# solvithrastar/MultiMesh

Hardware: AMD Instinct MI355X
Metric: interpolated points/sec, 10M->10M 3D mesh, 1 scalar field (higher is better)
Workload: dtype f64; 1 GPU; metric: hex8 3D 10077696 source nodes -> 10077696 targets in all, 10077696 on rank 0 (n_src=216, n_tgt=216 per side, jittered unit cube), 1 field component(s), k=20; targets: ONE 216^3 = 10077696-node target mesh (jitter seed 7); targets_per_gpu=10077696, targets_total=10077696, knn_kernel=lane, parallelism=single GPU

## Files before the change

### include/multimesh_hip.h

```cpp
#ifndef MULTIMESH_HIP_H
#define MULTIMESH_HIP_H

#include <stddef.h>
#include <stdint.h>

#ifdef __cplusplus
extern "C" {
#endif

#define MM_OK 0
#define MM_ERR_ARG (-1)
#define MM_ERR_HIP (-2)
#define MM_ERR_NODEVICE (-3)
#define MM_ERR_ALLOC (-4)
#define MM_ERR_UNSUPPORTED (-5)

#define MM_KNN_MAX_K 64


void centroid(long long ndim, long long nelem, long long npointsperelem,
              long long *connectivity, double *points, double *centroid);

long long triLinearInterpolator(long long nelem_to_search, long long npoints,
                                long long *nearest_element_indices, long long *connectivity,
// ... 129 lines not shown

int64_t mm_interpolate_hex8(mm_context *ctx, const double *nodes_d, int64_t nnodes,
                            const int64_t *connectivity_d, int64_t nelem, const double *points_d,
                            int64_t npoints, const double *fields_d, int64_t ncomp,
                            int64_t nelem_to_search, double *out_d, int64_t *enc_d, double *w_d);

typedef struct mm_source mm_source;
int mm_source_create(mm_context *ctx, const double *nodes_d, int64_t nnodes, const int64_t *connectivity_d, int64_t nelem,
                     mm_source **out);
void mm_source_destroy(mm_context *ctx, mm_source *source);
int64_t mm_interpolate_hex8_on(mm_context *ctx, const mm_source *source, const double *points_d, int64_t npoints,
                               const double *fields_d, int64_t ncomp, int64_t nelem_to_search, double *out_d,
                               int64_t *enc_d, double *w_d);

int64_t mm_interpolate_hex8_host(mm_context *ctx, const double *nodes_h, int64_t nnodes,
                                 const int64_t *connectivity_h, int64_t nelem, const double *points_h,
                                 int64_t npoints, const double *fields_h, int64_t ncomp,
                                 int64_t nelem_to_search, double *out_h, int64_t *enc_h, double *w_h);

int mm_set_lazy_lists(mm_context *ctx, int on);

#define MM_FP_EXACT 0
#define MM_FP_TOL 1
int mm_set_fp_mode(mm_context *ctx, int mode);
int mm_get_fp_mode(mm_context *ctx);
int mm_last_locate_stats(mm_context *ctx, long long *out4);
#define MM_KNN_RAN_LANE 1
#define MM_KNN_RAN_STRIP 2
#define MM_KNN_RAN_CELL 4
#define MM_KNN_RAN_LIST 8
#define MM_KNN_RAN_GENERIC 16
#define MM_KNN_RAN_LEVELS 32
#define MM_KNN_RAN_TREE 64
int mm_last_knn_kernels(mm_context *ctx, int *mask);

enum mm_stage {
    MM_STAGE_CENTROID = 0,
    MM_STAGE_KNN_BUILD = 1,
    MM_STAGE_KNN_QUERY = 2,
    MM_STAGE_LOCATE = 3,
    MM_STAGE_GATHER = 4,
    MM_STAGE_KNN_CELL = 5,
    MM_STAGE_LOCATE_PASS0 = 6,
    MM_STAGE_COUNT = 7
};
int mm_set_profiling(mm_context *ctx, int on);
int mm_last_timings(mm_context *ctx, double *ms, int n);

#ifdef __cplusplus
}
#endif
#endif
```

### multimesh_amd/csrc/mm_centroid.hip

```cpp
#include "mm_common.h"

template <int NDIM, int NPER>
__global__ __launch_bounds__(256) void centroid_kernel(i64 nelem, i64 nper_rt,
                                                       const i64 *__restrict__ conn,
                                                       const double *__restrict__ points,
                                                       double *__restrict__ out)
{
    const i64 e = (i64)blockIdx.x * blockDim.x + threadIdx.x;
    if (e >= nelem) return;
    const i64 nper = NPER > 0 ? NPER : nper_rt;
    const i64 *row = conn + e * nper;
    double acc[NDIM];
#pragma unroll
    for (int a = 0; a < NDIM; ++a) acc[a] = 0.;
    if (NPER > 0) {
        i64 id[NPER > 0 ? NPER : 1];
#pragma unroll
        for (int p = 0; p < NPER; ++p) id[p] = row[p];
#pragma unroll
        for (int p = 0; p < NPER; ++p) {
#pragma unroll
            for (int a = 0; a < NDIM; ++a) acc[a] = acc[a] + points[id[p] * NDIM + a];
        }
    } else {
        for (i64 p = 0; p < nper; ++p) {
            const i64 id = row[p];
#pragma unroll
            for (int a = 0; a < NDIM; ++a) acc[a] = acc[a] + points[id * NDIM + a];
        }
    }
    const double denom = (double)nper;
#pragma unroll
    for (int a = 0; a < NDIM; ++a) out[e * NDIM + a] = acc[a] / denom;
// ... 25 lines not shown
        double acc[3] = {0., 0., 0.};
#pragma unroll
        for (int p = 0; p < 8; ++p) {
#pragma unroll
            for (int a = 0; a < 3; ++a) acc[a] = acc[a] + points[id[p] * 3 + a];
        }
#pragma unroll
        for (int a = 0; a < 3; ++a) {
            const double c = acc[a] / 8.0;
            out[e * 3 + a] = c;
            mn[a] = fmin(mn[a], c);
            mx[a] = fmax(mx[a], c);
        }
    }
#pragma unroll
    for (int a = 0; a < 3; ++a)
        for (int off = 32; off > 0; off >>= 1) {
            mn[a] = fmin(mn[a], __shfl_xor(mn[a], off));
            mx[a] = fmax(mx[a], __shfl_xor(mx[a], off));
        }
    const int wave = threadIdx.x >> 6;
    if ((threadIdx.x & 63) == 0)
#pragma unroll
        for (int a = 0; a < 3; ++a) {
            s_box[a][wave] = mn[a];
            s_box[3 + a][wave] = mx[a];
        }
    __syncthreads();
    if (threadIdx.x < 6) {
        double v = s_box[threadIdx.x][0];
        for (int w = 1; w < 256 / 64; ++w) v = threadIdx.x < 3 ? fmin(v, s_box[threadIdx.x][w]) : fmax(v, s_box[threadIdx.x][w]);
        partial[(i64)blockIdx.x * 6 + threadIdx.x] = v;
    }
}

int mm_launch_centroid_bbox(mm_context *ctx, i64 nelem, const i64 *conn, const double *points, double *out,
                            double *partial, int nblocks)
{
    if (nelem == 0) return MM_OK;
    hipLaunchKernelGGL(centroid_bbox_kernel, dim3((unsigned)nblocks), dim3(256), 0, ctx->stream, nelem, conn, points,
                       out, partial);
    MM_HIP_CHECK(hipGetLastError());
    return MM_OK;
}

int mm_launch_centroid(mm_context *ctx, i64 ndim, i64 nelem, i64 nper, const i64 *conn,
                       const double *points, double *out)
{
    if (nelem == 0) return MM_OK;
    const int block = 256;
    const i64 grid = (nelem + block - 1) / block;
    MM_REQUIRE(grid < (i64)0x7fffffff, "too many elements for one launch");
    dim3 g((unsigned)grid), b(block);
    if (ndim == 3 && nper == 8)
        hipLaunchKernelGGL((centroid_kernel<3, 8>), g, b, 0, ctx->stream, nelem, nper, conn, points, out);
    else if (ndim == 3)
        hipLaunchKernelGGL((centroid_kernel<3, 0>), g, b, 0, ctx->stream, nelem, nper, conn, points, out);
    else if (ndim == 2 && nper == 4)
        hipLaunchKernelGGL((centroid_kernel<2, 4>), g, b, 0, ctx->stream, nelem, nper, conn, points, out);
    else if (ndim == 2)
        hipLaunchKernelGGL((centroid_kernel<2, 0>), g, b, 0, ctx->stream, nelem, nper, conn, points, out);
    else
        hipLaunchKernelGGL((centroid_kernel<1, 0>), g, b, 0, ctx->stream, nelem, nper, conn, points, out);
    MM_HIP_CHECK(hipGetLastError());
    return MM_OK;
}
// ... 16 lines not shown
```

### multimesh_amd/csrc/mm_common.h

```cpp
#pragma once

#include <hip/hip_runtime.h>
#include <stdint.h>
#include <stdio.h>

#include "multimesh_hip.h"

typedef long long i64;

void mm_set_error(int code, const char *fmt, ...);

#define MM_HIP_CHECK(expr)                                                              \
    do {                                                                                \
        hipError_t _e = (expr);                                                         \
        if (_e != hipSuccess) {                                                         \
            mm_set_error(MM_ERR_HIP, "%s:%d: %s -> %s", __FILE__, __LINE__, #expr,      \
                         hipGetErrorString(_e));                                        \
            return MM_ERR_HIP;                                                          \
        }                                                                               \
    } while (0)

#define MM_REQUIRE(cond, msg)                                                           \
    do {                                                                                \
        if (!(cond)) {                                                                  \
// ... 37 lines not shown
    MM_BUF_L_PTS,
    MM_BUF_LOC_SLOW,
    MM_BUF_TREE_KEYS,
    MM_BUF_TREE_XYZ,
    MM_BUF_TREE_LEVEL,
    MM_BUF_TREE_COARSE,
    MM_BUF_TREE_DOWN,
    MM_BUF_LEVELS,
    MM_BUF_SAMPLE_POINTS = MM_BUF_LEVELS + 2 * 8,
    MM_BUF_COUNT
};

struct mm_context {
    int device = 0;
    hipStream_t stream = nullptr;
    mm_scratch scratch;
    void *buf_ptr[MM_BUF_COUNT] = {};
    size_t buf_cap[MM_BUF_COUNT] = {};
    i64 *d_counters = nullptr;
    i64 *h_counters = nullptr;
    int profiling = 0;
    int lazy_lists = 1;
    int fp_mode = 0;
    hipEvent_t ev_begin[MM_STAGE_COUNT];
    hipEvent_t ev_end[MM_STAGE_COUNT];
    bool ev_used[MM_STAGE_COUNT];
    bool ev_created = false;
    hipEvent_t ev_misc = nullptr;
    struct {
        bool valid = false;
        i64 nsrc = 0;
        double box[6] = {0, 0, 0, 0, 0, 0};
        int stat_shift = -1;
        int misses = 0;
        long long calls_guessed = 0;
    } grid_guess;
    struct {
        bool valid = false;
        i64 npts = 0, ncells = 0;
        bool dense = false;
    } lane_hint;
    int knn_kernels = 0;
    int *abort_flags = nullptr;
    hipStream_t copy_stream = nullptr;
    hipEvent_t ev_copy[3] = {nullptr, nullptr, nullptr};
};

int mm_scratch_begin(mm_context *ctx, size_t total);
void *mm_scratch_take(mm_context *ctx, size_t bytes);
static inline size_t mm_round256(size_t b) { return (b + 255) & ~(size_t)255; }
static inline size_t mm_fill_span(size_t b) { return mm_guard_alloc() ? b : mm_round256(b); }

int mm_zero_async(mm_context *ctx, void *dst_d, size_t bytes);

int mm_mirror_async(mm_context *ctx, long long *dst_pinned, const long long *src_d, int n);

int mm_buffer_get(mm_context *ctx, int slot, size_t bytes, void **out);

void mm_stage_reset(mm_context *ctx);
void mm_stage_begin(mm_context *ctx, int stage);
void mm_stage_end(mm_context *ctx, int stage);

constexpr int kMmStatSlot = 32, kMmBoxSlot = 48, kMmAbortSlot = 24;

__device__ __forceinline__ bool mm_aborted(const int *__restrict__ abort6)
{
    if (!abort6) return false;
    const int4 a = *reinterpret_cast<const int4 *>(abort6);
    const int2 b = *reinterpret_cast<const int2 *>(abort6 + 4);
    return (a.x | a.y | a.z | a.w | b.x | b.y) != 0;
}

int mm_launch_centroid(mm_context *ctx, i64 ndim, i64 nelem, i64 nper, const i64 *conn,
                       const double *points, double *out);
int mm_launch_centroid_bbox(mm_context *ctx, i64 nelem, const i64 *conn, const double *points, double *out,
                            double *partial, int nblocks);
struct mm_knn_index;
struct mm_lazy_lists {
    const mm_knn_index *index;
    i64 k_full;
    int *nn_full;
};
int mm_launch_locate_hex8(mm_context *ctx, i64 k, i64 npoints, const void *nn, bool nn_is_int32,
                          const i64 *conn, i64 nelem, int conn_is_exodus, i64 *enc, const double *nodes,
                          double *w, const double *pts, i64 *d_nfailed, int zero_failed,
                          const double *fields, i64 nnodes, i64 ncomp, double *out,
                          const mm_lazy_lists *lazy, const double *tsorted = nullptr);
#define MM_LONG_LIST_MIN 32768
int mm_knn_query_list_impl(mm_context *ctx, const mm_knn_index *ix, const double *pts_d, i64 npts, i64 k,
                           int *idx_d, const int *list, const int *list_count, i64 list_len_hint);
int mm_launch_gather(mm_context *ctx, const double *fields, i64 nsrc, i64 ncomp, const i64 *ids,
                     const double *w, i64 npoints, i64 P, double *out, int out_point_major);

struct mm_knn_tree {
    double lo[3] = {0, 0, 0};
    double size = 1.0;
    double scale = 1.0;
    unsigned long long *keys = nullptr;
    double *xyz = nullptr;
    unsigned char *level = nullptr;
    int *coarse = nullptr;
    bool borrowed = false;
};
// ... 17 lines not shown
```

### multimesh_amd/csrc/mm_knn.hip

```cpp
#include <math.h>
#include <stdlib.h>

#include <new>
#include <type_traits>

#include "mm_common.h"
#include <cstring>

int mm_exclusive_scan_int(mm_context *ctx, const int *counts, i64 n, int *start, int *tile_sums);
size_t mm_radix_sort_scratch(i64 n);
int mm_radix_sort_pairs(mm_context *ctx, unsigned long long *ka, unsigned long long *kb, unsigned *va, unsigned *vb, i64 n,
                        int first_shift, int end_shift, void *scratch, bool *in_a);

namespace {
#include "mm_knn_grid.inc.h"
#include "mm_knn_rings.inc.h"
#include "mm_knn_tiles.inc.h"
#include "mm_knn_tree.inc.h"
#include "mm_knn_lane.inc.h"

__global__ __launch_bounds__(kBlock) void target_scatter_kernel(const int *__restrict__ rank_of, i64 npts,
                                                                const double *__restrict__ pts, int ndim, GridParams g,
                                                                const int *__restrict__ start,
                                                                double *__restrict__ tsorted,
                                                                const int *__restrict__ list,
                                                                const int *__restrict__ list_count)
{
    const i64 t = (i64)blockIdx.x * blockDim.x + threadIdx.x;
    if (t >= (list ? (i64)*list_count : npts)) return;
    const i64 p = list ? (i64)list[t] : t;
    const double x = pts[p * ndim], y = ndim > 1 ? pts[p * ndim + 1] : 0.0, z = ndim > 2 ? pts[p * ndim + 2] : 0.0;
    const i64 pos = (i64)start[cell_of_point(x, y, z, g)] + rank_of[t];
    store_record(tsorted + pos * kRec, x, y, z, (int)p);
}

constexpr int kLaneMaxK = 20;
struct LaneWork {
    int Z;
    int T, W;
// ... 298 lines not shown
{
    const unsigned gpts = (unsigned)((npts + kBlock - 1) / kBlock);
    const int ntiles = (int)((ncells + kScanTile - 1) / kScanTile);
    if (!list && ncells <= kHistCells && npts >= 64 * ncells)
        hipLaunchKernelGGL(cell_count_hist_kernel, dim3(256), dim3(kHistBlock), 0, ctx->stream, pts_d, npts, ndim, gl,
                           (int)ncells, cell_of, counts);
    else
        hipLaunchKernelGGL(cell_count_kernel, dim3(gpts), dim3(kBlock), 0, ctx->stream, pts_d, npts, ndim, gl, cell_of,
                           counts, list, list_count);
    hipLaunchKernelGGL(scan_tile_sums_kernel, dim3(ntiles), dim3(kBlock), 0, ctx->stream, counts, ncells, tile_sums,
                       (unsigned long long *)nullptr, 0);
    launch_scan_tail(ctx, counts, ncells, tile_sums, ntiles, start);
    hipLaunchKernelGGL(target_scatter_kernel, dim3(gpts), dim3(kBlock), 0, ctx->stream, cell_of, npts, pts_d, ndim, gl,
                       start, tsorted, list, list_count);
    MM_HIP_CHECK(hipGetLastError());
    return MM_OK;
}

static int build_level(mm_context *ctx, const double *src_d, i64 nsrc, int ndim, const double *box, double per_cell,
                       bool use_context_buffers, int level, int *level_extra, mm_knn_index **out,
                       double *sparse_share = nullptr, bool stat_dirty = true, const GuessedBuild *guessed = nullptr)
{
    static_assert(kMaxLevels - 1 <= 8, "mm_buffer_slot reserves 8 pairs for the denser levels");
    const int slot_cells = level == 0 ? (int)MM_BUF_CELL_START : (int)MM_BUF_LEVELS + 2 * (level - 1);
    const int slot_xyz = level == 0 ? (int)MM_BUF_SORTED_XYZ : (int)MM_BUF_LEVELS + 2 * (level - 1) + 1;
    *out = nullptr;
    mm_knn_index *ix = new (std::nothrow) mm_knn_index();
    if (!ix) {
        mm_set_error(MM_ERR_ALLOC, "out of host memory");
        return MM_ERR_ALLOC;
    }
    ix->nsrc = nsrc;
    ix->ndim = ndim;
    int live = 0;
    grid_layout(box, nsrc, ndim, per_cell, ix, &live);
    const i64 ncells = ix->ncells;
    const GridParams g = params_of(ix);

    hipError_t e = hipSuccess;
    if (use_context_buffers) {
        ix->borrowed = true;
        int brc = mm_buffer_get(ctx, slot_cells, (size_t)(ncells + 1) * sizeof(int), (void **)&ix->cell_start);
        if (brc == MM_OK)
            brc = mm_buffer_get(ctx, slot_xyz, (size_t)(nsrc + 1) * kRec * sizeof(double), (void **)&ix->sorted_xyz);
        if (brc != MM_OK) {
            free_index(ix);
            return brc;
        }
    } else {
        e = mm_raw_alloc(ctx->device, (void **)&ix->cell_start, (size_t)(ncells + 1) * sizeof(int));
        if (e == hipSuccess)
            e = mm_raw_alloc(ctx->device, (void **)&ix->sorted_xyz, (size_t)(nsrc + 1) * kRec * sizeof(double));
        if (e != hipSuccess) {
            mm_set_error(MM_ERR_ALLOC, "kNN index allocation failed: %s", hipGetErrorString(e));
            free_index(ix);
            return MM_ERR_ALLOC;
        }
    }
    const int ntiles = (int)((ncells + kScanTile - 1) / kScanTile);
    size_t need = mm_round256((size_t)(nsrc > 0 ? nsrc : 1) * sizeof(int)) +
                  mm_round256((size_t)(ncells + 1) * sizeof(int)) +
                  mm_round256((size_t)ntiles * sizeof(int)) + 4096;
    int rc = mm_scratch_begin(ctx, need);
    if (rc != MM_OK) { free_index(ix); return rc; }
    int *cell_of = (int *)mm_scratch_take(ctx, (size_t)(nsrc > 0 ? nsrc : 1) * sizeof(int));
    int *counts = (int *)mm_scratch_take(ctx, (size_t)(ncells + 1) * sizeof(int));
    int *tile_sums = (int *)mm_scratch_take(ctx, (size_t)ntiles * sizeof(int));
    if (!cell_of || !counts || !tile_sums) {
        mm_set_error(MM_ERR_ALLOC, "scratch carve failed");
        free_index(ix);
        return MM_ERR_ALLOC;
    }
    rc = mm_zero_async(ctx, counts, mm_fill_span((size_t)(ncells + 1) * sizeof(int)));
    if (rc != MM_OK) { free_index(ix); return rc; }
    const unsigned gsrc = (unsigned)((nsrc + kBlock - 1) / kBlock);
    if (guessed)
        {
            GuessBox gb6;
            for (int q = 0; q < 6; ++q) gb6.v[q] = box[q];
            hipLaunchKernelGGL(bbox_final_kernel, dim3(6), dim3(kBlock), 0, ctx->stream, guessed->box_partial, guessed->box_nblocks,
                               reinterpret_cast<double *>(ctx->h_counters + kBoxSlot),
                               reinterpret_cast<long long *>(ctx->d_counters + kStatSlot), gb6,
                               reinterpret_cast<int *>(ctx->d_counters + kMmAbortSlot));
        }
    if (nsrc > 0)
        hipLaunchKernelGGL(cell_count_kernel, dim3(gsrc), dim3(kBlock), 0, ctx->stream, src_d, nsrc, ndim, g, cell_of,
                           counts, (const int *)nullptr, (const int *)nullptr);
    const bool want_stat = level_extra != nullptr && nsrc >= kLevelMinSources && live > 0;
    const int sample_shift = (ncells + kBlock - 1) / kBlock >= 1024 ? 4 : 0;
    if (level_extra) *level_extra = 0;
    i64 *stat = ctx->d_counters + kStatSlot;
    if (want_stat && stat_dirty) e = hipMemsetAsync(stat, 0, 16 * sizeof(i64), ctx->stream);
    if (e == hipSuccess)
        hipLaunchKernelGGL(scan_tile_sums_kernel, dim3(ntiles), dim3(kBlock), 0, ctx->stream, counts, ncells, tile_sums,
                           want_stat ? (unsigned long long *)stat : (unsigned long long *)nullptr, sample_shift);
    launch_scan_tail(ctx, counts, ncells, tile_sums, ntiles, ix->cell_start,
                     want_stat ? (const long long *)stat : (const long long *)nullptr,
                     (long long *)(ctx->h_counters + kStatSlot), want_stat ? kMaxLevels : 0);
    if (want_stat) {
        if (e == hipSuccess) e = hipEventRecord(ctx->ev_misc, ctx->stream);
        if (e != hipSuccess) {
            mm_set_error(MM_ERR_HIP, "grid statistic: %s", hipGetErrorString(e));
            free_index(ix);
            return MM_ERR_HIP;
        }
    }
    if (nsrc > 0)
        hipLaunchKernelGGL(cell_scatter_kernel, dim3(gsrc), dim3(kBlock), 0, ctx->stream, src_d, nsrc, ndim, g, cell_of,
                           ix->cell_start, ix->sorted_xyz);
    e = hipGetLastError();
    if (e != hipSuccess) {
        mm_set_error(MM_ERR_HIP, "kNN build launch: %s", hipGetErrorString(e));
        free_index(ix);
        return MM_ERR_HIP;
    }
    if (guessed) *guessed->stat_shift = want_stat ? sample_shift : -1;
// ... 74 lines not shown
    {
        const int mode = tree_mode();
        bool cube = ndim == 3 && nsrc >= kLevelMinSources;
        for (int a = 0; a < 3 && cube; ++a) cube = box[3 + a] - box[a] > 0.0 && isfinite(box[3 + a] - box[a]);
        const bool deepest = (extra & (1 << (kMaxLevels - 2))) != 0, mesh_graded = (box_partial_d != nullptr || hex8_centroids) && extra != 0;
        if (cube && (mode == 1 || (mode == -1 && (deepest || mesh_graded) && max_levels > 1))) {
            rc = tree_build(ctx, head, src_d, nsrc, box, use_context_buffers);
            if (rc != MM_OK) {
                free_index(head);
                return rc;
            }
            extra = 0x10000;
        }
    }
    mm_knn_index *tail = head;
    for (int l = 1; l < max_levels; ++l) {
        per_cell /= kLevelRatio;
        if (!(extra & (1 << (l - 1)))) continue;
        if ((double)nsrc / per_cell > (double)kLevelMaxCells) break;
        mm_knn_index *lvl = nullptr;
        rc = build_level(ctx, src_d, nsrc, (int)ndim, box, per_cell, use_context_buffers, l, nullptr, &lvl);
        if (rc != MM_OK) {
            free_index(head);
            return rc;
        }
        tail->fine = lvl;
        tail = lvl;
    }
    *out = head;
    if (use_context_buffers && box_partial_d && ndim == 3) {
        ctx->grid_guess.valid = !head->fine && extra == 0 && per_cell_level0 == kDefaultPerCell && max_levels > 1;
        ctx->grid_guess.nsrc = nsrc;
        for (int q = 0; q < 6; ++q) ctx->grid_guess.box[q] = box[q];
    }
    return MM_OK;
}

int mm_knn_build_guessed(mm_context *ctx, const double *cen, i64 nelem, const double *box_partial, int box_nblocks,
                         mm_knn_index **out)
{
    *out = nullptr;
    GuessedBuild gb;
    gb.box_partial = box_partial;
    gb.box_nblocks = box_nblocks;
    gb.stat_shift = &ctx->grid_guess.stat_shift;
    int extra = 0;
    double sparse = 0.0;
    return build_level(ctx, cen, nelem, 3, ctx->grid_guess.box, kDefaultPerCell, true, 0, &extra, out, &sparse,
                       false, &gb);
}

bool mm_knn_guess_confirmed(mm_context *ctx)
{
    const double *h_box = reinterpret_cast<const double *>(ctx->h_counters + kBoxSlot);
    if (memcmp(h_box, ctx->grid_guess.box, 6 * sizeof(double)) != 0) return false;
    if (ctx->grid_guess.stat_shift < 0) return true;
    double sparse_count = 0.0;
    const int extra = stat_verdict(ctx, ctx->grid_guess.nsrc, ctx->grid_guess.stat_shift, &sparse_count);
    return extra == 0 && !(sparse_count / (double)ctx->grid_guess.nsrc > kSparseShare);
}


static TreeParams tree_params_of(const mm_knn_tree *tr)
{
    TreeParams tp;
    tp.lox = tr->lo[0];
    tp.loy = tr->lo[1];
    tp.loz = tr->lo[2];
    tp.scale = tr->scale;
    tp.size = tr->size;
    return tp;
}

static int tree_mode()
{
    const char *env = getenv("MM_KNN_TREE");
    return env ? (atoi(env) == 0 ? 0 : 1) : -1;
}

static int tree_build(mm_context *ctx, mm_knn_index *ix, const double *src_d, i64 nsrc, const double *box,
                      bool use_context_buffers)
{
    mm_knn_tree *tr = new (std::nothrow) mm_knn_tree();
    if (!tr) {
        mm_set_error(MM_ERR_ALLOC, "out of host memory");
        return MM_ERR_ALLOC;
    }
    double ext = 0.0;
// ... 486 lines not shown
```

### multimesh_amd/csrc/mm_knn_grid.inc.h

```cpp


constexpr int kBlock = 256;
constexpr double kDefaultPerCell = 8.0;
constexpr int kMaxCellsPerAxis = 1024;
constexpr double kLevelRatio = 2.0;
constexpr int kMaxLevels = 9;
constexpr int kLevelCount[kMaxLevels - 1] = {15, 19, 38, 77, 154, 307, 614, 1229};
constexpr double kLevelShare = 0.02;
constexpr int kSparseCount = 5;
constexpr double kSparseShare = 0.25;
constexpr i64 kLevelMinSources = 4096;
constexpr i64 kLevelMaxCells = (i64)1 << 27;
constexpr int kListKeepMax = 24;
constexpr i64 kLongListMin = MM_LONG_LIST_MIN;
constexpr int kSplitTargets = 128;
constexpr int kMaxSplit = 64;
constexpr int kStatSlot = kMmStatSlot;
static_assert(kMaxLevels <= 16, "the level statistic has 16 counter slots");
constexpr int kBoxSlot = kMmBoxSlot;

struct GridParams {
    int nx, ny, nz;
    double lox, loy, loz;
    double hx, hy, hz;
    double ihx, ihy, ihz;
};

__global__ __launch_bounds__(kBlock) void bbox_partial_kernel(const double *__restrict__ src, i64 nsrc,
                                                              int ndim, double *__restrict__ partial)
{
    __shared__ double smin[3][kBlock / 64];
    __shared__ double smax[3][kBlock / 64];
    double mn[3] = {INFINITY, INFINITY, INFINITY};
    double mx[3] = {-INFINITY, -INFINITY, -INFINITY};
    for (i64 e = (i64)blockIdx.x * blockDim.x + threadIdx.x; e < nsrc; e += (i64)gridDim.x * blockDim.x) {
        for (int a = 0; a < ndim; ++a) {
            const double v = src[e * ndim + a];
            mn[a] = fmin(mn[a], v);
            mx[a] = fmax(mx[a], v);
        }
    }
    for (int a = 0; a < 3; ++a) {
        for (int off = 32; off > 0; off >>= 1) {
            mn[a] = fmin(mn[a], __shfl_xor(mn[a], off));
            mx[a] = fmax(mx[a], __shfl_xor(mx[a], off));
        }
    }
    const int wave = threadIdx.x >> 6;
    if ((threadIdx.x & 63) == 0)
        for (int a = 0; a < 3; ++a) {
            smin[a][wave] = mn[a];
            smax[a][wave] = mx[a];
        }
    __syncthreads();
    if (threadIdx.x == 0) {
        for (int a = 0; a < 3; ++a) {
            double lo = smin[a][0], hi = smax[a][0];
            for (int wv = 1; wv < kBlock / 64; ++wv) {
                lo = fmin(lo, smin[a][wv]);
                hi = fmax(hi, smax[a][wv]);
            }
            partial[blockIdx.x * 6 + a] = lo;
            partial[blockIdx.x * 6 + 3 + a] = hi;
        }
    }
}

struct GuessBox {
    double v[6];
};
__global__ __launch_bounds__(kBlock) void bbox_final_kernel(const double *__restrict__ partial, int nblocks,
                                                             double *__restrict__ out, long long *__restrict__ stat16,
                                                             GuessBox guess = GuessBox(), int *__restrict__ mismatch6 = nullptr)
{
    __shared__ double s_part[kBlock / 64];
    const int a = blockIdx.x;
    if (stat16 && a == 0 && threadIdx.x < 16) stat16[threadIdx.x] = 0;
    const double init = a < 3 ? INFINITY : -INFINITY;
    double v[8];
#pragma unroll
    for (int u = 0; u < 8; ++u) v[u] = init;
    for (int b = threadIdx.x; b < nblocks; b += 8 * kBlock) {
#pragma unroll
        for (int u = 0; u < 8; ++u) {
            const int bb = b + kBlock * u;
            const double p = bb < nblocks ? partial[bb * 6 + a] : init;
            v[u] = a < 3 ? fmin(v[u], p) : fmax(v[u], p);
        }
    }
    double r = init;
#pragma unroll
    for (int u = 0; u < 8; ++u) r = a < 3 ? fmin(r, v[u]) : fmax(r, v[u]);
    for (int off = 32; off > 0; off >>= 1) {
        const double o = __shfl_xor(r, off);
        r = a < 3 ? fmin(r, o) : fmax(r, o);
    }
    if ((threadIdx.x & 63) == 0) s_part[threadIdx.x >> 6] = r;
    __syncthreads();
    if (threadIdx.x == 0) {
        for (int wv = 1; wv < kBlock / 64; ++wv) r = a < 3 ? fmin(r, s_part[wv]) : fmax(r, s_part[wv]);
        out[a] = r;
        if (mismatch6) mismatch6[a] = r == guess.v[a] ? 0 : 1;
    }
}

__device__ __forceinline__ int cell_coord(double x, double lo, double ih, int n)
{
    double t = (x - lo) * ih;
    t = fmin(fmax(t, 0.0), (double)(n - 1));
    return (int)t;
}

__device__ __forceinline__ int count_and_rank(int c, bool live, int *__restrict__ counts)
{
    const int lane = threadIdx.x & 63;
    const int prev = __shfl_up(c, 1);
    const bool head = lane == 0 || c != prev;
    const unsigned long long heads = __ballot(head);
    const unsigned long long upto = heads & (~0ull >> (63 - lane));
    const int head_lane = 63 - __clzll((long long)upto);
    const unsigned long long after = lane == 63 ? 0ull : heads & (~0ull << (lane + 1));
    int base = 0;
    if (head && live) {
        const int next_head = after ? __ffsll((long long)after) - 1 : 64;
        base = atomicAdd(&counts[c], next_head - lane);
    }
    base = __shfl(base, head_lane);
    return base + (lane - head_lane);
}

__device__ __forceinline__ int cell_of_point(double x, double y, double z, const GridParams &g)
{
    const int cx = cell_coord(x, g.lox, g.ihx, g.nx);
    const int cy = cell_coord(y, g.loy, g.ihy, g.ny);
    const int cz = cell_coord(z, g.loz, g.ihz, g.nz);
    return (cx * g.ny + cy) * g.nz + cz;
}

__global__ __launch_bounds__(kBlock) void cell_count_kernel(const double *__restrict__ src, i64 nsrc, int ndim,
                                                            GridParams g, int *__restrict__ rank_of,
                                                            int *__restrict__ counts, const int *__restrict__ list,
                                                            const int *__restrict__ list_count)
{
    const i64 e = (i64)blockIdx.x * blockDim.x + threadIdx.x;
    const bool live = e < (list ? (i64)*list_count : nsrc);
    int c = -1;
    if (live) {
        const i64 p = list ? (i64)list[e] : e;
        c = cell_of_point(src[p * ndim], ndim > 1 ? src[p * ndim + 1] : 0.0, ndim > 2 ? src[p * ndim + 2] : 0.0, g);
    }
    const int rank = count_and_rank(c, live, counts);
    if (live) rank_of[e] = rank;
}

constexpr int kHistBlock = 1024;
constexpr int kHistCells = 16384;
__global__ __launch_bounds__(kHistBlock) void cell_count_hist_kernel(const double *__restrict__ src, i64 nsrc, int ndim,
                                                                     GridParams g, int ncells, int *__restrict__ rank_of,
                                                                     int *__restrict__ counts)
{
    __shared__ int s_bin[kHistCells];
    for (int t = threadIdx.x; t < ncells; t += kHistBlock) s_bin[t] = 0;
    __syncthreads();
    const i64 chunks = (nsrc + kHistBlock - 1) / kHistBlock;
    const i64 c_lo = chunks * blockIdx.x / gridDim.x, c_hi = chunks * (blockIdx.x + 1) / gridDim.x;
    for (i64 ch = c_lo; ch < c_hi; ++ch) {
        const i64 e = ch * kHistBlock + threadIdx.x;
        const bool live = e < nsrc;
        int c = -1;
// ... 128 lines not shown
        s += v[i];
    }
    int total;
    int excl = block_exclusive_scan(s, &total) + tile_base;
    for (int i = 0; i < kScanItems; ++i) {
        if (base + i < n) start[base + i] = excl;
        excl += v[i];
    }
    if (blockIdx.x == gridDim.x - 1 && threadIdx.x == kBlock - 1) start[n] = excl;
}

__global__ __launch_bounds__(kBlock) void scan_apply_kernel(const int *__restrict__ counts, i64 n,
                                                            const int *__restrict__ tile_offsets,
                                                            int *__restrict__ start)
{
    const i64 base = (i64)blockIdx.x * kScanTile + (i64)threadIdx.x * kScanItems;
    int v[kScanItems];
    int s = 0;
    for (int i = 0; i < kScanItems; ++i) {
        v[i] = base + i < n ? counts[base + i] : 0;
        s += v[i];
    }
    int total;
    int excl = block_exclusive_scan(s, &total) + tile_offsets[blockIdx.x];
    for (int i = 0; i < kScanItems; ++i) {
        if (base + i < n) {
            start[base + i] = excl;
        }
        excl += v[i];
    }
    if (blockIdx.x == gridDim.x - 1 && threadIdx.x == kBlock - 1) start[n] = excl;
}

constexpr int kRec = 4;

__device__ __forceinline__ void store_record(double *__restrict__ rec, double x, double y, double z, int id)
{
    double2 *r2 = reinterpret_cast<double2 *>(rec);
    r2[0] = make_double2(x, y);
    r2[1] = make_double2(z, __longlong_as_double((long long)id));
}

__device__ __forceinline__ int record_id(double w) { return (int)__double_as_longlong(w); }

__global__ __launch_bounds__(kBlock) void cell_scatter_kernel(const double *__restrict__ src, i64 nsrc, int ndim,
                                                              GridParams g, const int *__restrict__ rank_of,
                                                              const int *__restrict__ start,
                                                              double *__restrict__ sorted_rec)
{
    const i64 e = (i64)blockIdx.x * blockDim.x + threadIdx.x;
    if (e >= nsrc) return;
    const double x = src[e * ndim], y = ndim > 1 ? src[e * ndim + 1] : 0.0, z = ndim > 2 ? src[e * ndim + 2] : 0.0;
    const i64 pos = (i64)start[cell_of_point(x, y, z, g)] + rank_of[e];
    store_record(sorted_rec + pos * kRec, x, y, z, (int)e);
}


constexpr int kWave = 64;
constexpr int kHistBuckets = 64;
constexpr int kTileCap = 256;
constexpr int kMaxGroups = 8;
constexpr int kSlots = kTileCap / kMaxGroups;

__device__ __forceinline__ int group_scan(int v, int sl, int S)
{
    for (int d = 1; d < S; d <<= 1) {
        const int t = __shfl_up(v, d, S);
        if (sl >= d) v += t;
    }
    return v;
}

__device__ __forceinline__ void wave_sync()
{
    __builtin_amdgcn_fence(__ATOMIC_RELEASE, "wavefront");
    __builtin_amdgcn_wave_barrier();
    __builtin_amdgcn_fence(__ATOMIC_ACQUIRE, "wavefront");
// ... 2 lines not shown
```

### multimesh_amd/csrc/mm_pipeline.hip

```cpp
#include <cstdlib>
#include <mutex>
#include <new>

#include "mm_common.h"

int mm_knn_build_impl(mm_context *ctx, const double *src_d, i64 nsrc, i64 ndim, mm_knn_index **out,
                      bool use_context_buffers, const double *box_partial_d, int box_nblocks, bool hex8_centroids = false);
int mm_knn_query_impl(mm_context *ctx, const mm_knn_index *ix, const double *pts_d, i64 npts, i64 k, void *idx_d,
                      double *dist_d, bool idx_is_int32);
int mm_knn_query_sorted_impl(mm_context *ctx, const mm_knn_index *ix, const double *pts_d, i64 npts, i64 k, int *idx_d,
                             const double **tsorted_out);
void mm_clear_status(void);
int mm_knn_build_guessed(mm_context *ctx, const double *cen, i64 nelem, const double *box_partial, int box_nblocks,
                         mm_knn_index **out);
bool mm_knn_guess_confirmed(mm_context *ctx);

static const int64_t kLazyK = 8;
static const int kBoxBlocks = 2048;
static const int64_t kFuseGatherMaxComp = 3;

struct mm_host_feed {
    const void *src[4];
    void *dst[4];
    size_t bytes[4];
};

static int feed_upload(mm_context *ctx, const mm_host_feed *feed, int first, int last, int event)
{
    for (int a = first; a <= last; ++a)
        if (feed->bytes[a])
            MM_HIP_CHECK(hipMemcpyAsync(feed->dst[a], feed->src[a], feed->bytes[a], hipMemcpyHostToDevice, ctx->copy_stream));
    MM_HIP_CHECK(hipEventRecord(ctx->ev_copy[event], ctx->copy_stream));
    MM_HIP_CHECK(hipStreamWaitEvent(ctx->stream, ctx->ev_copy[event], 0));
    return MM_OK;
}

struct mm_source {
    const double *nodes = nullptr;
    i64 nnodes = 0;
    const i64 *conn = nullptr;
    i64 nelem = 0;
    double *centroids = nullptr;
    mm_knn_index *index = nullptr;
    int device = 0;
};

static int64_t interpolate_hex8_impl(mm_context *ctx, const double *nodes_d, int64_t nnodes,
// ... 35 lines not shown
    int *nn_full = nullptr;
    const double *tsorted = nullptr;
    mm_lazy_lists lazy;
    if (!resident) {
        rc = mm_buffer_get(ctx, MM_BUF_CENTROID, (size_t)nelem * 3 * sizeof(double), (void **)&cen);
        if (rc == MM_OK) rc = mm_buffer_get(ctx, MM_BUF_BOX_PARTIAL, (size_t)kBoxBlocks * 6 * sizeof(double), (void **)&box_partial);
    }
    if (rc == MM_OK) rc = mm_buffer_get(ctx, MM_BUF_NN, (size_t)npoints * (size_t)kq * sizeof(int), (void **)&nn);
    if (rc == MM_OK && kq < k)
        rc = mm_buffer_get(ctx, MM_BUF_NN_FULL, (size_t)npoints * (size_t)k * sizeof(int), (void **)&nn_full);
    const bool want_values = out_d && ncomp > 0;
    const bool fuse_gather = want_values && ncomp <= kFuseGatherMaxComp;
    if (!(enc && w)) {
        enc = nullptr;
        w = nullptr;
        if (want_values && !fuse_gather) {
            if (rc == MM_OK) rc = mm_buffer_get(ctx, MM_BUF_ENC, (size_t)npoints * 8 * sizeof(i64), (void **)&enc);
            if (rc == MM_OK) rc = mm_buffer_get(ctx, MM_BUF_W, (size_t)npoints * 8 * sizeof(double), (void **)&w);
        }
    }
    if (rc != MM_OK) { result = rc; goto done; }


    static const bool guess_on = !(getenv("MM_GRID_GUESS") && atoi(getenv("MM_GRID_GUESS")) == 0);
    guessed = guess_on && ctx->grid_guess.valid && ctx->grid_guess.nsrc == nelem && ctx->grid_guess.misses < 2 &&
              !getenv("MM_KNN_LEVELS") && !resident;
again:
    ctx->abort_flags = nullptr;
    if (resident) {
        index = resident->index;
        goto query;
    }
    if (feed && (rc = feed_upload(ctx, feed, 0, 1, 0)) != MM_OK) { result = rc; goto done; }
    mm_stage_begin(ctx, MM_STAGE_CENTROID);
    rc = mm_launch_centroid_bbox(ctx, nelem, (const i64 *)conn_d, nodes_d, cen, box_partial, kBoxBlocks);
    mm_stage_end(ctx, MM_STAGE_CENTROID);
    if (rc != MM_OK) { result = rc; goto done; }

    mm_stage_begin(ctx, MM_STAGE_KNN_BUILD);
    ctx->abort_flags = nullptr;
    if (guessed) {
        ++ctx->grid_guess.calls_guessed;
        ctx->abort_flags = reinterpret_cast<int *>(ctx->d_counters + kMmAbortSlot);
        rc = mm_knn_build_guessed(ctx, cen, nelem, box_partial, kBoxBlocks, &index);
    } else {
        rc = mm_knn_build_impl(ctx, cen, nelem, 3, &index, true, box_partial, kBoxBlocks);
    }
    mm_stage_end(ctx, MM_STAGE_KNN_BUILD);
    if (rc != MM_OK) { result = rc; goto done; }

query:
    if (feed && (rc = feed_upload(ctx, feed, 2, 2, 1)) != MM_OK) { result = rc; goto done; }
    mm_stage_begin(ctx, MM_STAGE_KNN_QUERY);
    rc = mm_knn_query_sorted_impl(ctx, index, points_d, npoints, kq, nn, kq < k ? &tsorted : nullptr);
    mm_stage_end(ctx, MM_STAGE_KNN_QUERY);
    if (rc != MM_OK) { result = rc; goto done; }

    if (feed && (rc = feed_upload(ctx, feed, 3, 3, 2)) != MM_OK) { result = rc; goto done; }
    mm_stage_begin(ctx, MM_STAGE_LOCATE);
    lazy.index = index;
    lazy.k_full = k;
    lazy.nn_full = nn_full;
    rc = mm_launch_locate_hex8(ctx, kq, npoints, nn, true, (const i64 *)conn_d, nelem, 1, enc,
                               nodes_d, w, points_d, ctx->d_counters, 1,
                               fuse_gather ? fields_d : nullptr, nnodes, ncomp, out_d,
                               kq < k ? &lazy : nullptr, tsorted);
    mm_stage_end(ctx, MM_STAGE_LOCATE);
    if (rc != MM_OK) { result = rc; goto done; }
    if (want_values && !fuse_gather) {
        mm_stage_begin(ctx, MM_STAGE_GATHER);
        rc = mm_launch_gather(ctx, fields_d, nnodes, ncomp, enc, w, npoints, 8, out_d, 1);
        mm_stage_end(ctx, MM_STAGE_GATHER);
        if (rc != MM_OK) { result = rc; goto done; }
    }

    rc = mm_mirror_async(ctx, (long long *)ctx->h_counters, (const long long *)ctx->d_counters, 1);
    if (rc != MM_OK) { result = rc; goto done; }
    e = hipStreamSynchronize(ctx->stream);
    if (e != hipSuccess) MM_PIPE_FAIL(MM_ERR_HIP, hipGetErrorString(e));
    if (guessed && !mm_knn_guess_confirmed(ctx)) {
        ctx->grid_guess.valid = false;
        ++ctx->grid_guess.misses;
        guessed = false;
        ctx->abort_flags = nullptr;
        mm_knn_destroy(nullptr, index);
        index = nullptr;
        feed = nullptr;
        mm_stage_reset(ctx);
        goto again;
    }
    result = ctx->h_counters[0];
    if (guessed && ctx->grid_guess.misses > 0 && (ctx->grid_guess.calls_guessed & 63) == 0) --ctx->grid_guess.misses;

done:
    ctx->abort_flags = nullptr;
    if (result < 0) (void)hipStreamSynchronize(ctx->stream);
    if (index && !resident) mm_knn_destroy(nullptr, index);
    return result;
#undef MM_PIPE_FAIL
}

extern "C" int mm_debug_grid_guess(mm_context *ctx, long long *out4)
{
    MM_REQUIRE(ctx != nullptr && out4 != nullptr, "null argument");
    out4[0] = ctx->grid_guess.valid ? 1 : 0;
    out4[1] = ctx->grid_guess.misses;
    out4[2] = ctx->grid_guess.calls_guessed;
    out4[3] = ctx->grid_guess.nsrc;
    return MM_OK;
}

extern "C" int64_t mm_interpolate_hex8(mm_context *ctx, const double *nodes_d, int64_t nnodes,
                                       const int64_t *conn_d, int64_t nelem, const double *points_d,
                                       int64_t npoints, const double *fields_d, int64_t ncomp, int64_t k,
                                       double *out_d, int64_t *enc_d, double *w_d)
{
    return interpolate_hex8_impl(ctx, nodes_d, nnodes, conn_d, nelem, points_d, npoints, fields_d, ncomp, k, out_d,
                                 enc_d, w_d, nullptr);
}

extern "C" int mm_source_create(mm_context *ctx, const double *nodes_d, int64_t nnodes, const int64_t *conn_d, int64_t nelem,
                                mm_source **out)
{
    MM_REQUIRE(ctx != nullptr && out != nullptr, "null argument");
// ... 305 lines not shown
```

### multimesh_amd/device.py

```python
from __future__ import annotations

import ctypes as C

import numpy as np

from . import helpers as H
from .helpers import MM_FP_EXACT, MM_FP_TOL, MM_KNN_MAX_K, STAGES, MultiMeshHipError, check, load_lib

KNN_KERNELS = ("lane", "strip", "cell", "list", "generic", "levels", "tree")

_NP2ITEM = {np.dtype(np.float64): 8, np.dtype(np.int64): 8, np.dtype(np.int32): 4, np.dtype(np.uint8): 1}


class DeviceArray:

    def __init__(self, ctx, ptr, shape, dtype, owner=True, keepalive=None):
        self.ctx = ctx
        self.ptr = int(ptr)
        self.shape = tuple(int(s) for s in shape)
        self.dtype = np.dtype(dtype)
        self._owner = owner
        self._keepalive = keepalive

    @property
    def nbytes(self):
        return int(np.prod(self.shape, dtype=np.int64)) * self.dtype.itemsize

    @property
    def size(self):
        return int(np.prod(self.shape, dtype=np.int64))

    def data_ptr(self):
        return self.ptr

    def numpy(self):
        out = np.empty(self.shape, dtype=self.dtype)
        if out.nbytes:
            check(self.ctx.lib.mm_copy_d2h(self.ctx.handle, out.ctypes.data, self.ptr, out.nbytes), "mm_copy_d2h")
        return out

    def rows(self, start, stop):
        row_bytes = self.nbytes // max(self.shape[0], 1) if self.shape[0] else 0
# ... 828 lines not shown
```

Baseline: 2.899 billion points/s.

## Fuse centroid computation with cell scatter using speculative cached cell layout

When the previous call's grid guess was confirmed, a new one-pass build runs. It computes element centroids and scatters them directly into cell-sorted records. It does this against the previous call's cell_start offsets, which skips the separate centroid write, cell count, scan and scatter kernels. A cursor-check kernel compares the per-cell counts against the cached offsets and raises an abort flag on mismatch. On a mismatch the host falls back to the full rebuild. This adds a verification kernel and widens the abort-flag check, and a wrong speculation costs a full recompute.

```diff
diff --git a/include/multimesh_hip.h b/include/multimesh_hip.h
--- a/include/multimesh_hip.h
+++ b/include/multimesh_hip.h
@@ -185,6 +185,7 @@
 #define MM_KNN_RAN_GENERIC 16
 #define MM_KNN_RAN_LEVELS 32
 #define MM_KNN_RAN_TREE 64
+#define MM_KNN_RAN_ONE_PASS 128
 int mm_last_knn_kernels(mm_context *ctx, int *mask);
 
 enum mm_stage {
diff --git a/multimesh_amd/csrc/mm_centroid.hip b/multimesh_amd/csrc/mm_centroid.hip
--- a/multimesh_amd/csrc/mm_centroid.hip
+++ b/multimesh_amd/csrc/mm_centroid.hip
@@ -1,4 +1,5 @@
 #include "mm_common.h"
+#include "mm_grid_cell.h"
 
 template <int NDIM, int NPER>
 __global__ __launch_bounds__(256) void centroid_kernel(i64 nelem, i64 nper_rt,
@@ -90,6 +91,86 @@
         for (int w = 1; w < 256 / 64; ++w) v = threadIdx.x < 3 ? fmin(v, s_box[threadIdx.x][w]) : fmax(v, s_box[threadIdx.x][w]);
         partial[(i64)blockIdx.x * 6 + threadIdx.x] = v;
     }
+}
+
+__global__ __launch_bounds__(256) void centroid_sort_kernel(i64 nelem, const i64 *__restrict__ conn,
+                                                            const double *__restrict__ points, GridParams g,
+                                                            const int *__restrict__ guess_start, int *__restrict__ cursor,
+                                                            double *__restrict__ sorted_rec, double *__restrict__ partial)
+{
+    __shared__ double s_box[6][256 / 64];
+    double mn[3] = {INFINITY, INFINITY, INFINITY}, mx[3] = {-INFINITY, -INFINITY, -INFINITY};
+    const i64 stride = (i64)gridDim.x * blockDim.x;
+    const int lane = threadIdx.x & 63;
+    i64 e = (i64)blockIdx.x * blockDim.x + threadIdx.x;
+    i64 idn[8];
+    {
+        const i64 *row = conn + (e < nelem ? e : 0) * 8;
+#pragma unroll
+        for (int p = 0; p < 8; ++p) idn[p] = row[p];
+    }
+    for (; e - lane < nelem; e += stride) {
+        const bool live = e < nelem;
+        i64 id[8];
+#pragma unroll
+        for (int p = 0; p < 8; ++p) id[p] = idn[p];
+        {
+            const i64 *row = conn + (e + stride < nelem ? e + stride : (live ? e : 0)) * 8;
+#pragma unroll
+            for (int p = 0; p < 8; ++p) idn[p] = row[p];
+        }
+        double acc[3] = {0., 0., 0.};
+#pragma unroll
+        for (int p = 0; p < 8; ++p) {
+#pragma unroll
+            for (int a = 0; a < 3; ++a) acc[a] = acc[a] + points[id[p] * 3 + a];
+        }
+        double c[3];
+#pragma unroll
+        for (int a = 0; a < 3; ++a) {
+            c[a] = acc[a] / 8.0;
+            if (live) {
+                mn[a] = fmin(mn[a], c[a]);
+                mx[a] = fmax(mx[a], c[a]);
+            }
+        }
+        const int cell = live ? cell_of_point(c[0], c[1], c[2], g) : -1;
+        const int rank = count_and_rank(cell, live, cursor);
+        if (live) {
+            const int first = guess_start[cell], room = guess_start[cell + 1] - first;
+            const i64 pos = (i64)first + rank;
+            if (rank >= 0 && rank < room && pos >= 0 && pos < nelem) store_record(sorted_rec + pos * kRec, c[0], c[1], c[2], (int)e);
+        }
+    }
+#pragma unroll
+    for (int a = 0; a < 3; ++a)
+        for (int off = 32; off > 0; off >>= 1) {
+            mn[a] = fmin(mn[a], __shfl_xor(mn[a], off));
+            mx[a] = fmax(mx[a], __shfl_xor(mx[a], off));
+        }
+    const int wave = threadIdx.x >> 6;
+    if (lane == 0)
+#pragma unroll
+        for (int a = 0; a < 3; ++a) {
+            s_box[a][wave] = mn[a];
+            s_box[3 + a][wave] = mx[a];
+        }
+    __syncthreads();
+    if (threadIdx.x < 6) {
+        double v = s_box[threadIdx.x][0];
+        for (int w = 1; w < 256 / 64; ++w) v = threadIdx.x < 3 ? fmin(v, s_box[threadIdx.x][w]) : fmax(v, s_box[threadIdx.x][w]);
+        partial[(i64)blockIdx.x * 6 + threadIdx.x] = v;
+    }
+}
+
+int mm_launch_centroid_sort(mm_context *ctx, i64 nelem, const i64 *conn, const double *points, const GridParams &g,
+                            const int *guess_start, int *cursor, double *sorted_rec, double *partial, int nblocks)
+{
+    if (nelem == 0) return MM_OK;
+    hipLaunchKernelGGL(centroid_sort_kernel, dim3((unsigned)nblocks), dim3(256), 0, ctx->stream, nelem, conn, points, g,
+                       guess_start, cursor, sorted_rec, partial);
+    MM_HIP_CHECK(hipGetLastError());
+    return MM_OK;
 }
 
 int mm_launch_centroid_bbox(mm_context *ctx, i64 nelem, const i64 *conn, const double *points, double *out,
diff --git a/multimesh_amd/csrc/mm_common.h b/multimesh_amd/csrc/mm_common.h
--- a/multimesh_amd/csrc/mm_common.h
+++ b/multimesh_amd/csrc/mm_common.h
@@ -93,6 +93,7 @@
         i64 nsrc = 0;
         double box[6] = {0, 0, 0, 0, 0, 0};
         int stat_shift = -1;
+        bool cells_ok = false;
         int misses = 0;
         long long calls_guessed = 0;
     } grid_guess;
@@ -123,13 +124,14 @@
 void mm_stage_end(mm_context *ctx, int stage);
 
 constexpr int kMmStatSlot = 32, kMmBoxSlot = 48, kMmAbortSlot = 24;
+constexpr int kMmCountsBadSlot = 54;
 
 __device__ __forceinline__ bool mm_aborted(const int *__restrict__ abort6)
 {
     if (!abort6) return false;
     const int4 a = *reinterpret_cast<const int4 *>(abort6);
-    const int2 b = *reinterpret_cast<const int2 *>(abort6 + 4);
-    return (a.x | a.y | a.z | a.w | b.x | b.y) != 0;
+    const int4 b = *reinterpret_cast<const int4 *>(abort6 + 4);
+    return (a.x | a.y | a.z | a.w | b.x | b.y | b.z | b.w) != 0;
 }
 
 int mm_launch_centroid(mm_context *ctx, i64 ndim, i64 nelem, i64 nper, const i64 *conn,
diff --git a/multimesh_amd/csrc/mm_grid_cell.h b/multimesh_amd/csrc/mm_grid_cell.h
--- /dev/null
+++ b/multimesh_amd/csrc/mm_grid_cell.h
@@ -0,0 +1,57 @@
+#pragma once
+
+#include "mm_common.h"
+
+struct GridParams {
+    int nx, ny, nz;
+    double lox, loy, loz;
+    double hx, hy, hz;
+    double ihx, ihy, ihz;
+};
+
+__device__ __forceinline__ int cell_coord(double x, double lo, double ih, int n)
+{
+    double t = (x - lo) * ih;
+    t = fmin(fmax(t, 0.0), (double)(n - 1));
+    return (int)t;
+}
+
+__device__ __forceinline__ int count_and_rank(int c, bool live, int *__restrict__ counts)
+{
+    const int lane = threadIdx.x & 63;
+    const int prev = __shfl_up(c, 1);
+    const bool head = lane == 0 || c != prev;
+    const unsigned long long heads = __ballot(head);
+    const unsigned long long upto = heads & (~0ull >> (63 - lane));
+    const int head_lane = 63 - __clzll((long long)upto);
+    const unsigned long long after = lane == 63 ? 0ull : heads & (~0ull << (lane + 1));
+    int base = 0;
+    if (head && live) {
+        const int next_head = after ? __ffsll((long long)after) - 1 : 64;
+        base = atomicAdd(&counts[c], next_head - lane);
+    }
+    base = __shfl(base, head_lane);
+    return base + (lane - head_lane);
+}
+
+__device__ __forceinline__ int cell_of_point(double x, double y, double z, const GridParams &g)
+{
+    const int cx = cell_coord(x, g.lox, g.ihx, g.nx);
+    const int cy = cell_coord(y, g.loy, g.ihy, g.ny);
+    const int cz = cell_coord(z, g.loz, g.ihz, g.nz);
+    return (cx * g.ny + cy) * g.nz + cz;
+}
+
+constexpr int kRec = 4;
+
+__device__ __forceinline__ void store_record(double *__restrict__ rec, double x, double y, double z, int id)
+{
+    double2 *r2 = reinterpret_cast<double2 *>(rec);
+    r2[0] = make_double2(x, y);
+    r2[1] = make_double2(z, __longlong_as_double((long long)id));
+}
+
+__device__ __forceinline__ int record_id(double w) { return (int)__double_as_longlong(w); }
+
+int mm_launch_centroid_sort(mm_context *ctx, i64 nelem, const i64 *conn, const double *points, const GridParams &g,
+                            const int *guess_start, int *cursor, double *sorted_rec, double *partial, int nblocks);
diff --git a/multimesh_amd/csrc/mm_knn.hip b/multimesh_amd/csrc/mm_knn.hip
--- a/multimesh_amd/csrc/mm_knn.hip
+++ b/multimesh_amd/csrc/mm_knn.hip
@@ -5,6 +5,7 @@
 #include <type_traits>
 
 #include "mm_common.h"
+#include "mm_grid_cell.h"
 #include <cstring>
 
 int mm_exclusive_scan_int(mm_context *ctx, const int *counts, i64 n, int *start, int *tile_sums);
@@ -369,6 +370,7 @@
     }
     ix->nsrc = nsrc;
     ix->ndim = ndim;
+    if (use_context_buffers && level == 0) ctx->grid_guess.cells_ok = false;
     int live = 0;
     grid_layout(box, nsrc, ndim, per_cell, ix, &live);
     const i64 ncells = ix->ncells;
@@ -418,7 +420,8 @@
             hipLaunchKernelGGL(bbox_final_kernel, dim3(6), dim3(kBlock), 0, ctx->stream, guessed->box_partial, guessed->box_nblocks,
                                reinterpret_cast<double *>(ctx->h_counters + kBoxSlot),
                                reinterpret_cast<long long *>(ctx->d_counters + kStatSlot), gb6,
-                               reinterpret_cast<int *>(ctx->d_counters + kMmAbortSlot));
+                               reinterpret_cast<int *>(ctx->d_counters + kMmAbortSlot),
+                               reinterpret_cast<long long *>(ctx->h_counters + kMmCountsBadSlot));
         }
     if (nsrc > 0)
         hipLaunchKernelGGL(cell_count_kernel, dim3(gsrc), dim3(kBlock), 0, ctx->stream, src_d, nsrc, ndim, g, cell_of,
@@ -559,6 +562,7 @@
         ctx->grid_guess.valid = !head->fine && extra == 0 && per_cell_level0 == kDefaultPerCell && max_levels > 1;
         ctx->grid_guess.nsrc = nsrc;
         for (int q = 0; q < 6; ++q) ctx->grid_guess.box[q] = box[q];
+        ctx->grid_guess.cells_ok = ctx->grid_guess.valid;
     }
     return MM_OK;
 }
@@ -577,10 +581,70 @@
                        false, &gb);
 }
 
+int mm_knn_build_one_pass(mm_context *ctx, const i64 *conn, const double *nodes, i64 nelem, double *box_partial,
+                          int box_nblocks, mm_knn_index **out)
+{
+    *out = nullptr;
+    mm_knn_index *ix = new (std::nothrow) mm_knn_index();
+    if (!ix) {
+        mm_set_error(MM_ERR_ALLOC, "out of host memory");
+        return MM_ERR_ALLOC;
+    }
+    ix->nsrc = nelem;
+    ix->ndim = 3;
+    grid_layout(ctx->grid_guess.box, nelem, 3, kDefaultPerCell, ix, nullptr);
+    const i64 ncells = ix->ncells;
+    const GridParams g = params_of(ix);
+    ix->borrowed = true;
+    int rc = mm_buffer_get(ctx, MM_BUF_CELL_START, (size_t)(ncells + 1) * sizeof(int), (void **)&ix->cell_start);
+    if (rc == MM_OK) rc = mm_buffer_get(ctx, MM_BUF_SORTED_XYZ, (size_t)(nelem + 1) * kRec * sizeof(double), (void **)&ix->sorted_xyz);
+    if (rc == MM_OK) rc = mm_scratch_begin(ctx, mm_round256((size_t)(ncells + 1) * sizeof(int)) + 1024);
+    int *cursor = rc == MM_OK ? (int *)mm_scratch_take(ctx, (size_t)(ncells + 1) * sizeof(int)) : nullptr;
+    if (rc == MM_OK && !cursor) {
+        mm_set_error(MM_ERR_ALLOC, "scratch carve failed");
+        rc = MM_ERR_ALLOC;
+    }
+    if (rc != MM_OK) {
+        free_index(ix);
+        return rc;
+    }
+    mm_stage_begin(ctx, MM_STAGE_CENTROID);
+    rc = mm_zero_async(ctx, cursor, mm_fill_span((size_t)(ncells + 1) * sizeof(int)));
+    if (rc == MM_OK)
+        rc = mm_launch_centroid_sort(ctx, nelem, conn, nodes, g, ix->cell_start, cursor, ix->sorted_xyz, box_partial, box_nblocks);
+    mm_stage_end(ctx, MM_STAGE_CENTROID);
+    if (rc != MM_OK) {
+        free_index(ix);
+        return rc;
+    }
+    mm_stage_begin(ctx, MM_STAGE_KNN_BUILD);
+    GuessBox gb6;
+    for (int q = 0; q < 6; ++q) gb6.v[q] = ctx->grid_guess.box[q];
+    int *flags = reinterpret_cast<int *>(ctx->d_counters + kMmAbortSlot);
+    long long *counts_bad_h = reinterpret_cast<long long *>(ctx->h_counters + kMmCountsBadSlot);
+    hipLaunchKernelGGL(bbox_final_kernel, dim3(6), dim3(kBlock), 0, ctx->stream, (const double *)box_partial, box_nblocks,
+                       reinterpret_cast<double *>(ctx->h_counters + kBoxSlot), (long long *)nullptr, gb6, flags, counts_bad_h);
+    const i64 want = (ncells + kBlock - 1) / kBlock;
+    hipLaunchKernelGGL(cursor_check_kernel, dim3((unsigned)(want > 1024 ? 1024 : want)), dim3(kBlock), 0, ctx->stream,
+                       (const int *)cursor, (const int *)ix->cell_start, ncells, flags, counts_bad_h);
+    mm_stage_end(ctx, MM_STAGE_KNN_BUILD);
+    const hipError_t e = hipGetLastError();
+    if (e != hipSuccess) {
+        mm_set_error(MM_ERR_HIP, "one-pass kNN build launch: %s", hipGetErrorString(e));
+        free_index(ix);
+        return MM_ERR_HIP;
+    }
+    ctx->grid_guess.stat_shift = -1;
+    ctx->knn_kernels |= MM_KNN_RAN_ONE_PASS;
+    *out = ix;
+    return MM_OK;
+}
+
 bool mm_knn_guess_confirmed(mm_context *ctx)
 {
     const double *h_box = reinterpret_cast<const double *>(ctx->h_counters + kBoxSlot);
     if (memcmp(h_box, ctx->grid_guess.box, 6 * sizeof(double)) != 0) return false;
+    if (ctx->h_counters[kMmCountsBadSlot] != 0) return false;
     if (ctx->grid_guess.stat_shift < 0) return true;
     double sparse_count = 0.0;
     const int extra = stat_verdict(ctx, ctx->grid_guess.nsrc, ctx->grid_guess.stat_shift, &sparse_count);
diff --git a/multimesh_amd/csrc/mm_knn_grid.inc.h b/multimesh_amd/csrc/mm_knn_grid.inc.h
--- a/multimesh_amd/csrc/mm_knn_grid.inc.h
+++ b/multimesh_amd/csrc/mm_knn_grid.inc.h
@@ -19,12 +19,6 @@
 static_assert(kMaxLevels <= 16, "the level statistic has 16 counter slots");
 constexpr int kBoxSlot = kMmBoxSlot;
 
-struct GridParams {
-    int nx, ny, nz;
-    double lox, loy, loz;
-    double hx, hy, hz;
-    double ihx, ihy, ihz;
-};
 
 __global__ __launch_bounds__(kBlock) void bbox_partial_kernel(const double *__restrict__ src, i64 nsrc,
                                                               int ndim, double *__restrict__ partial)
@@ -71,7 +65,8 @@
 };
 __global__ __launch_bounds__(kBlock) void bbox_final_kernel(const double *__restrict__ partial, int nblocks,
                                                              double *__restrict__ out, long long *__restrict__ stat16,
-                                                             GuessBox guess = GuessBox(), int *__restrict__ mismatch6 = nullptr)
+                                                             GuessBox guess = GuessBox(), int *__restrict__ mismatch6 = nullptr,
+                                                             long long *__restrict__ counts_bad_h = nullptr)
 {
     __shared__ double s_part[kBlock / 64];
     const int a = blockIdx.x;
@@ -101,40 +96,25 @@
         for (int wv = 1; wv < kBlock / 64; ++wv) r = a < 3 ? fmin(r, s_part[wv]) : fmax(r, s_part[wv]);
         out[a] = r;
         if (mismatch6) mismatch6[a] = r == guess.v[a] ? 0 : 1;
-    }
-}
-
-__device__ __forceinline__ int cell_coord(double x, double lo, double ih, int n)
-{
-    double t = (x - lo) * ih;
-    t = fmin(fmax(t, 0.0), (double)(n - 1));
-    return (int)t;
-}
-
-__device__ __forceinline__ int count_and_rank(int c, bool live, int *__restrict__ counts)
-{
-    const int lane = threadIdx.x & 63;
-    const int prev = __shfl_up(c, 1);
-    const bool head = lane == 0 || c != prev;
-    const unsigned long long heads = __ballot(head);
-    const unsigned long long upto = heads & (~0ull >> (63 - lane));
-    const int head_lane = 63 - __clzll((long long)upto);
-    const unsigned long long after = lane == 63 ? 0ull : heads & (~0ull << (lane + 1));
-    int base = 0;
-    if (head && live) {
-        const int next_head = after ? __ffsll((long long)after) - 1 : 64;
-        base = atomicAdd(&counts[c], next_head - lane);
-    }
-    base = __shfl(base, head_lane);
-    return base + (lane - head_lane);
-}
-
-__device__ __forceinline__ int cell_of_point(double x, double y, double z, const GridParams &g)
-{
-    const int cx = cell_coord(x, g.lox, g.ihx, g.nx);
-    const int cy = cell_coord(y, g.loy, g.ihy, g.ny);
-    const int cz = cell_coord(z, g.loz, g.ihz, g.nz);
-    return (cx * g.ny + cy) * g.nz + cz;
+        if (mismatch6 && a == 0) {
+            mismatch6[6] = 0;
+            mismatch6[7] = 0;
+            if (counts_bad_h) *counts_bad_h = 0;
+        }
+    }
+}
+
+__global__ __launch_bounds__(kBlock) void cursor_check_kernel(const int *__restrict__ cursor, const int *__restrict__ start,
+                                                              i64 ncells, int *__restrict__ mismatch8,
+                                                              long long *__restrict__ counts_bad_h)
+{
+    bool bad = false;
+    for (i64 c = (i64)blockIdx.x * blockDim.x + threadIdx.x; c < ncells; c += (i64)gridDim.x * blockDim.x)
+        bad = bad || cursor[c] != start[c + 1] - start[c];
+    if (__any(bad) && (threadIdx.x & 63) == 0) {
+        mismatch8[6] = 1;
+        *counts_bad_h = 1;
+    }
 }
 
 __global__ __launch_bounds__(kBlock) void cell_count_kernel(const double *__restrict__ src, i64 nsrc, int ndim,
@@ -329,17 +309,6 @@
     if (blockIdx.x == gridDim.x - 1 && threadIdx.x == kBlock - 1) start[n] = excl;
 }
 
-constexpr int kRec = 4;
-
-__device__ __forceinline__ void store_record(double *__restrict__ rec, double x, double y, double z, int id)
-{
-    double2 *r2 = reinterpret_cast<double2 *>(rec);
-    r2[0] = make_double2(x, y);
-    r2[1] = make_double2(z, __longlong_as_double((long long)id));
-}
-
-__device__ __forceinline__ int record_id(double w) { return (int)__double_as_longlong(w); }
-
 __global__ __launch_bounds__(kBlock) void cell_scatter_kernel(const double *__restrict__ src, i64 nsrc, int ndim,
                                                               GridParams g, const int *__restrict__ rank_of,
                                                               const int *__restrict__ start,
diff --git a/multimesh_amd/csrc/mm_pipeline.hip b/multimesh_amd/csrc/mm_pipeline.hip
--- a/multimesh_amd/csrc/mm_pipeline.hip
+++ b/multimesh_amd/csrc/mm_pipeline.hip
@@ -13,6 +13,8 @@
 void mm_clear_status(void);
 int mm_knn_build_guessed(mm_context *ctx, const double *cen, i64 nelem, const double *box_partial, int box_nblocks,
                          mm_knn_index **out);
+int mm_knn_build_one_pass(mm_context *ctx, const i64 *conn, const double *nodes, i64 nelem, double *box_partial,
+                          int box_nblocks, mm_knn_index **out);
 bool mm_knn_guess_confirmed(mm_context *ctx);
 
 static const int64_t kLazyK = 8;
@@ -114,6 +116,13 @@
         goto query;
     }
     if (feed && (rc = feed_upload(ctx, feed, 0, 1, 0)) != MM_OK) { result = rc; goto done; }
+    if (guessed && ctx->grid_guess.cells_ok) {
+        ++ctx->grid_guess.calls_guessed;
+        ctx->abort_flags = reinterpret_cast<int *>(ctx->d_counters + kMmAbortSlot);
+        rc = mm_knn_build_one_pass(ctx, (const i64 *)conn_d, nodes_d, nelem, box_partial, kBoxBlocks, &index);
+        if (rc != MM_OK) { result = rc; goto done; }
+        goto query;
+    }
     mm_stage_begin(ctx, MM_STAGE_CENTROID);
     rc = mm_launch_centroid_bbox(ctx, nelem, (const i64 *)conn_d, nodes_d, cen, box_partial, kBoxBlocks);
     mm_stage_end(ctx, MM_STAGE_CENTROID);
@@ -162,6 +171,7 @@
     if (e != hipSuccess) MM_PIPE_FAIL(MM_ERR_HIP, hipGetErrorString(e));
     if (guessed && !mm_knn_guess_confirmed(ctx)) {
         ctx->grid_guess.valid = false;
+        ctx->grid_guess.cells_ok = false;
         ++ctx->grid_guess.misses;
         guessed = false;
         ctx->abort_flags = nullptr;
@@ -172,6 +182,7 @@
         goto again;
     }
     result = ctx->h_counters[0];
+    if (guessed) ctx->grid_guess.cells_ok = true;
     if (guessed && ctx->grid_guess.misses > 0 && (ctx->grid_guess.calls_guessed & 63) == 0) --ctx->grid_guess.misses;
 
 done:
diff --git a/multimesh_amd/device.py b/multimesh_amd/device.py
--- a/multimesh_amd/device.py
+++ b/multimesh_amd/device.py
@@ -7,7 +7,7 @@
 from . import helpers as H
 from .helpers import MM_FP_EXACT, MM_FP_TOL, MM_KNN_MAX_K, STAGES, MultiMeshHipError, check, load_lib
 
-KNN_KERNELS = ("lane", "strip", "cell", "list", "generic", "levels", "tree")
+KNN_KERNELS = ("lane", "strip", "cell", "list", "generic", "levels", "tree", "one_pass")
 
 _NP2ITEM = {np.dtype(np.float64): 8, np.dtype(np.int64): 8, np.dtype(np.int32): 4, np.dtype(np.uint8): 1}
 
```

After: 2.998 billion points/s (median of 6 runs). 1.03x the previous value.
